# 2lambda123/CliMA-Oceananigans.jl

Hardware: AMD Instinct MI355X
Metric: cell-updates/sec per time_step!, 256^3 Nonhydrostatic WENO5 (higher is better)
Workload: dtype f64

## Files before the change

### clima-oceananigans.jl_amd/csrc/compat.h

```cpp
#pragma once

#include <cmath>
#include <cstddef>
#include <cstdint>
#include <cstdio>
#include <cstdlib>
#include <cstring>

#ifndef OCN_HOST_EMU
#include <hip/hip_runtime.h>
#include <hipfft/hipfft.h>

#define OCN_DEVFN __device__ __forceinline__

extern thread_local int g_ocn_dry;

struct ocn_launch_error {
  hipError_t err;
  char what[200];
};
extern thread_local ocn_launch_error g_ocn_launch_err;
static inline void ocn_note_error(hipError_t e, const char* what) {
  if (e == hipSuccess || g_ocn_launch_err.err != hipSuccess) return;
  g_ocn_launch_err.err = e;
// ... 14 lines not shown

typedef __attribute__((address_space(3))) void ocn_lds_void;
typedef const __attribute__((address_space(1))) void ocn_glb_void;
__device__ __forceinline__ void ocn_glds16(const void* src_lane, void* dst_wave_base, int ) {
  __builtin_amdgcn_global_load_lds((ocn_glb_void*)src_lane, (ocn_lds_void*)dst_wave_base, 16, 0, 0);
}
__device__ __forceinline__ double ocn_shfl_next(double x) {
  union { double d; int i[2]; } a, b;
  a.d = x;
  b.i[0] = __builtin_amdgcn_update_dpp(0, a.i[0], 0x130, 0xf, 0xf, false);
  b.i[1] = __builtin_amdgcn_update_dpp(0, a.i[1], 0x130, 0xf, 0xf, false);
  return b.d;
}
__device__ __forceinline__ double ocn_shfl_xor16(double x) {
  union { double d; int i[2]; } a, b;
  a.d = x;
  const int lane = __builtin_amdgcn_mbcnt_hi(~0u, __builtin_amdgcn_mbcnt_lo(~0u, 0u));
  const int addr = (lane ^ 16) << 2;
  b.i[0] = __builtin_amdgcn_ds_bpermute(addr, a.i[0]);
  b.i[1] = __builtin_amdgcn_ds_bpermute(addr, a.i[1]);
  return b.d;
}
#define OCN_WAVE 64
#define OCN_LD_NT(p) __builtin_nontemporal_load(p)
#define OCN_ST_NT(p, v) __builtin_nontemporal_store((v), (p))
#define OCN_UNIFORM(x) __builtin_amdgcn_readfirstlane(x)
typedef const __attribute__((address_space(4))) double ocn_const_double;
#define OCN_SLOAD(p) (*(ocn_const_double*)(p))

#else
#include <chrono>
#include <condition_variable>
#include <mutex>
#include <thread>
#include <vector>

struct dim3 {
  unsigned x, y, z;
  dim3(unsigned a = 1, unsigned b = 1, unsigned c = 1) : x(a), y(b), z(c) {}
};
extern thread_local dim3 threadIdx, blockIdx, blockDim, gridDim;
#define g_ocn_dry 0
extern std::recursive_mutex g_emu_launch_mutex;

#define __global__
#define __device__
// ... 50 lines not shown
          for (unsigned ty = 0; ty < block.y; ++ty)
            for (unsigned tx = 0; tx < block.x; ++tx) {
              threadIdx = dim3(tx, ty, tz);
              kern(args...);
            }
      }
}

struct emu_barrier {
  std::mutex m;
  std::condition_variable cv;
  unsigned count = 0, n = 0, gen = 0;
  void wait() {
    std::unique_lock<std::mutex> lk(m);
    unsigned g = gen;
    if (++count == n) { count = 0; ++gen; cv.notify_all(); }
    else cv.wait(lk, [&] { return g != gen; });
  }
};
extern emu_barrier g_emu_barrier;
static inline void __syncthreads() { g_emu_barrier.wait(); }

#define OCN_WAVE 64
#define OCN_UNIFORM(x) (x)
#define OCN_SLOAD(p) (*(p))
#define OCN_LD_NT(p) (*(p))
#define OCN_ST_NT(p, v) ((void)(*(p) = (v)))
static inline void ocn_glds16(const void* src_lane, void* dst_wave_base, int lane) {
  memcpy((char*)dst_wave_base + 16 * lane, src_lane, 16);
}
extern double g_emu_shfl[4096];
static inline double ocn_shfl_xor16(double x) {
  const unsigned tid = threadIdx.x + blockDim.x * (threadIdx.y + blockDim.y * threadIdx.z);
  g_emu_shfl[tid] = x;
  g_emu_barrier.wait();
  const double y = g_emu_shfl[tid ^ 16];
  g_emu_barrier.wait();
  return y;
}
static inline double ocn_shfl_next(double x) {
  const unsigned tid = threadIdx.x + blockDim.x * (threadIdx.y + blockDim.y * threadIdx.z);
  const unsigned n = blockDim.x * blockDim.y * blockDim.z;
  g_emu_shfl[tid] = x;
  g_emu_barrier.wait();
  const double y = ((tid & 63) != 63 && tid + 1 < n) ? g_emu_shfl[tid + 1] : 0.0;
  g_emu_barrier.wait();
// ... 38 lines not shown
```

### clima-oceananigans.jl_amd/csrc/fused.hip

```cpp
#include "internal.h"

#define FUSED_MAX_THREADS 1024

struct FusedArgs {
  const double *u, *v, *w;
  const double *gmu, *gmv, *gmw;
  double *gnu, *gnv, *gnw;
  double *us, *vs, *ws;
  unsigned org;
  double dt, cn, cm;
  int use_m;
  int BYo;
  int ntiles;
  int ntx, BXo;
  int prio;
  double nu;
  int zlo, zhi;
  int zlo2, zhi2;
  int gran;
};

#ifndef OCN_HOST_EMU
#define OCN_SETPRIO(n) __builtin_amdgcn_s_setprio(n)
#else
// ... 874 lines not shown
  if (m->d.closure == OCN_CLOSURE_AMD || m->d.closure == OCN_CLOSURE_SMAG || m->d.coriolis_fplane || m->d.buoyancy != OCN_BUOYANCY_NONE) return false;
  if (tiled_blocker(m)) return false;
  if (getenv("OCNHIP_NO_FUSED")) return false;
  return true;
}

bool fused_available(const ocn_model* m) {
  if (m->stokes) return false;
  return fused_available_but_for_stokes(m);
}

static bool tend4_asel(const ocn_model* m, bool plain);

void fused_describe(const ocn_model* m, char* buf, size_t n) {
  const char* why = tiled_blocker(m);
  if (m->fast_path) {
    const size_t halo_bytes = (size_t)(3 + m->nt) * m->gd.Hz * m->u.sz * sizeof(double);
    const bool ov = m->g->dist && m->gd.Nz > 2 * m->gd.Hz + 2 &&
                    (m->knob_overlap >= 0 ? m->knob_overlap != 0 : (m->ctx->nranks > 1 && halo_bytes >= ((size_t)8 << 20)));
    const bool asel = tend4_asel(m, !(m->d.closure == OCN_CLOSURE_SCALAR && m->d.nu != 0.0));
    const char* pform = m->g->dist ? "" : pnhs_lazy(m) ? " (pressure written on demand)"
                        : m->pnhs_escaped ? " (pressure stored by every projection: its device pointer was handed out)"
                                          : " (pressure stored by every projection)";
    snprintf(buf, n, "all-in-one periodic path: k_tend4%s + fused Poisson passes + k_project%s%s", asel ? " (address-selected stencils)" : "",
             pform, !m->g->dist ? "" : ov ? "; z-slabs, halo planes travel under the next interior tendency launch"
                                   : "; z-slabs, halo exchange on the model's stream");
  }
  else if (m->bz_fast) snprintf(buf, n, "tiled advection + update (k_tend4, REST) on top of the %s other terms",
                                rest4_ok(m) ? "tiled kernel's (k_rest4)" : "general kernels'");
  else if (why) snprintf(buf, n, "general kernels: %s", why);
  else if (m->g->topo[0] == OCN_FLAT || m->g->topo[1] == OCN_FLAT) snprintf(buf, n, "general kernels: Flat x / y slices are outside the tiled kernels");
  else snprintf(buf, n, "general kernels (tiled path disabled or not applicable to this topology / decomposition)");
  if (m->stokes && fused_available_but_for_stokes(m)) {
    const size_t l = strlen(buf);
    snprintf(buf + l, n - l, "; not the all-in-one periodic path: Stokes drift terms are served by %s",
             rest4_ok(m) ? "k_rest4" : "the general kernel");
  }
  if (m->d.closure == OCN_CLOSURE_SMAG) {
    const size_t l = strlen(buf);
    snprintf(buf + l, n - l, "; nu_e: %s", smag_tiled_ok(m) ? "tiled kernel (k_smag_nu)" : "one thread per cell (k_smag_nu_cell)");
  }
}

int fused_cu_count(const ocn_model* m) {
  static int ncu = 0;
  if (!ncu) {
#ifndef OCN_HOST_EMU
    hipDeviceProp_t prop;
    ncu = (hipGetDeviceProperties(&prop, m->ctx->device) == hipSuccess) ? prop.multiProcessorCount : 256;
#else
    ncu = 8;
#endif
  }
  return ncu;
}

struct FusedShape {
  int bx, by;
  bool wide, small;
  int dma;
  bool asel;
  dim3 blk, grd;
};

void fused_read_knobs(ocn_model* m) {
  auto env = [](const char* n, int def) { const char* e = getenv(n); return e ? atoi(e) : def; };
  m->knob_fused_xt = env("OCNHIP_FUSED_XT", 0);
  m->knob_no_dma = env("OCNHIP_NO_LDS_DMA", 0);
  m->knob_no_tracer3 = env("OCNHIP_NO_TRACER3", 0);
  m->knob_xfft_team = env("OCNHIP_XFFT_TEAM", 0);
  m->knob_overlap = env("OCNHIP_OVERLAP", -1);
  m->knob_overlap_cus = env("OCNHIP_OVERLAP_CUS", 16);
  m->knob_graph = env("OCNHIP_NO_GRAPH", 0) ? 0 : 1;
  { const char* e = getenv("OCNHIP_PRIO"); m->knob_prio = e ? (int)strtol(e, nullptr, 0) : 0x20FF; }
  { const char* e = getenv("OCNHIP_LOCALITY"); m->knob_locality = e ? atoi(e) : 1; }
  m->knob_no_smag_tiled = env("OCNHIP_NO_SMAG_TILED", 0);
  m->knob_tend4_vsel = env("OCNHIP_TEND4_VSEL", 0);
  m->knob_eager_pressure = env("OCNHIP_EAGER_PRESSURE", 0);
}

static bool tend4_asel(const ocn_model* m, bool plain) {
  const GridDev& gd = m->gd;
  if (!plain || m->knob_tend4_vsel || gd.Nx > 256 || gd.xb || (m->knob_fused_xt == 1 && gd.Nx <= 57 * 4)) return false;
#ifdef OCN_HOST_EMU
  return gd.Nx <= 16;
#else
  return gd.Nx > 128;
#endif
}

static FusedShape fused_shape(const ocn_model* m, FusedArgs& a, bool plain = false) {
  const GridDev& gd = m->gd;
  FusedShape f;
// ... 364 lines not shown
```

### clima-oceananigans.jl_amd/csrc/internal.h

```cpp
#pragma once
#include <map>
#include <string>
#include <vector>

#include "../../include/ocnhip.h"
#include "compat.h"
#include "stencils.h"

#define OCN_NF (3 + OCN_MAX_TRACERS)
#define OCN_CLOSURE_SMAG 3

struct ProfPhase {
  std::vector<std::pair<hipEvent_t, hipEvent_t>> ev;
  double total_ms = 0;
  int64_t count = 0;
};

struct ocn_ctx {
  int device = 0;
  hipStream_t stream = nullptr;
  char err[512] = {0};
  bool profiling = false;
  std::map<std::string, ProfPhase> prof;
  std::string prof_only;
// ... 73 lines not shown
  double time = 0, previous_dt = INFINITY;
  int64_t iteration = 0;
  int stage = 1;
  double* d_red = nullptr;
  int fast_path = 0;
  int bz_fast = 0;
  double* amd_tab = nullptr;
  double smag_C = 0, smag_Cb = 0, smag_rPr[OCN_MAX_TRACERS] = {0};
  double* smag_tab = nullptr;
  int knob_no_smag_tiled = 0;
  double* phi_below = nullptr;
  double *ypack_s = nullptr, *ypack_r = nullptr;
  size_t ypack_n = 0;
  bool gn_alias_gm = false;
  bool pred_active = false;
  ocn_grid* own_grid = nullptr;
  int knob_fused_xt = 0, knob_no_dma = 0, knob_no_tracer3 = 0, knob_prio = 0x20FF;
  struct StepGraph { uint64_t key; int seen; void* exec; std::vector<uint64_t> words; };
  std::vector<StepGraph> graphs;
  int knob_overlap_cus = 16;
  int knob_overlap = -1;
  bool halo_inflight = false, halo2_inflight = false;
  bool pnhs_halo_stale = false;
  int knob_xfft_team = 0;
  int knob_graph = 1;
  int knob_tend4_vsel = 0;
  int knob_locality = 1;
  bool pnhs_deferred = false;
  bool pnhs_escaped = false;
  int knob_eager_pressure = 0;
  int stokes = 0;
  double* stokes_dev = nullptr;
  double* stokes_stage = nullptr;
  hipEvent_t stokes_ev[3] = {nullptr, nullptr, nullptr};
  bool graph_off = false;
  int64_t graph_replays = 0;
};
extern thread_local int g_ocn_capturing, g_ocn_capture_poison;
inline Field& pred_u(ocn_model* m) { return m->pred_active ? m->us : m->u; }
inline Field& pred_v(ocn_model* m) { return m->pred_active ? m->vs : m->v; }
inline Field& pred_w(ocn_model* m) { return m->pred_active ? m->ws : m->w; }
inline bool pnhs_lazy(const ocn_model* m) { return m->fast_path && !m->g->dist && !m->knob_eager_pressure && !m->pnhs_escaped; }

inline const double* stokes_slot(const ocn_model* m) {
  return m->stokes ? m->stokes_dev + (size_t)(m->stage - 1) * 6 * m->gd.Nz : nullptr;
}
// ... 35 lines not shown
bool fused_tracer3_ok(const ocn_model* m);
bool tracer_rest_shell(const ocn_model* m);
void launch_tracer3(ocn_model* m, double dt, double cn, double cm, int use_m, bool rest);
void launch_fused_tend_step(ocn_model* m, double dt, double cn, double cm, int use_m, int zlo = 0, int zhi = -1, int zlo2 = 0, int zhi2 = 0);
void launch_rhs_wrap(ocn_model* m, double dt, double* rhs);
void launch_project(ocn_model* m, double dt, const double* phi, bool store_p = true);
void launch_pressure_images(ocn_model* m, const double* phi);
void launch_tracer_steps(ocn_model* m, double dt, double cn, double cm, int use_m);
int fused_exchange_ws(ocn_model* m);
int fused_exchange_phi(ocn_model* m, const double* phi);
int poisson_run(ocn_model* m);

PoissonSolver* poisson_create(ocn_model* m);
void poisson_destroy(PoissonSolver* s);
int poisson_solve(ocn_model* m, double dt);
int poisson_solve_rhs(ocn_model* m, const double* rhs_dev, double* phi_dev);
double* poisson_rhs_buffer(PoissonSolver* s);

void* zsolve_create(ocn_ctx* ctx, const std::vector<double>& lx_half, const std::vector<double>& ly_local);
void zsolve_destroy(void* z);
void zsolve_run(ocn_ctx* ctx, void* z, void* spec, int Nz, const double* lz, double norm, long zero_col);
void yfft_run(ocn_ctx* ctx, void* z, void* spec, int Nxh, int Ny, int Nz, int inverse);
void xfft_rhs_run(ocn_model* m, void* z, void* spec, double dt, int extra_plane = 0);
bool poisson_local_wstar(const ocn_model* m);
bool fft_size_ok(int n);
bool zsolve_size_ok(int n);
bool poisson_custom_xy(const ocn_model* m);
int poisson_run_from_predictor(ocn_model* m, double dt);

void* zslab_create(ocn_ctx* ctx, const std::vector<double>& lx_half, const std::vector<double>& ly, int n, int R, int rank);
void zslab_destroy(void* z);
int zslab_run(ocn_ctx* ctx, void* z, void* spec, double dz2, double scale, const void* below = nullptr, void* phi_below = nullptr);
bool poisson_local_phi_below(const ocn_model* m);
const double* poisson_phi_below(const ocn_model* m);

int comm_exchange(ocn_ctx* c, const std::vector<CommOp>& sends, const std::vector<CommOp>& recvs, hipStream_t st = nullptr);
int comm_halo_exchange_z(ocn_model* m, Field** fs, int n, hipStream_t st = nullptr);
bool comm_can_overlap(const ocn_ctx* c);
int halo_settle(ocn_model* m);
int comm_halo_exchange_y(ocn_model* m, Field** fs, int n);
int comm_alltoall(ocn_ctx* c, const void* send, void* recv, size_t block_bytes);
void comm_destroy(ocn_ctx* c);

struct ProfScope {
  ocn_ctx* c;
  hipEvent_t a = nullptr, b = nullptr;
// ... 5 lines not shown
```

### clima-oceananigans.jl_amd/csrc/poisson.hip

```cpp
#include "internal.h"
#ifndef OCN_HOST_EMU
#define dry_hipfftExecD2Z(...) (g_ocn_dry ? HIPFFT_SUCCESS : hipfftExecD2Z(__VA_ARGS__))
#define dry_hipfftExecZ2D(...) (g_ocn_dry ? HIPFFT_SUCCESS : hipfftExecZ2D(__VA_ARGS__))
#define dry_hipfftExecZ2Z(...) (g_ocn_dry ? HIPFFT_SUCCESS : hipfftExecZ2Z(__VA_ARGS__))
#endif


#ifndef OCN_HOST_EMU
#include <rocblas/rocblas.h>
#endif
#include <complex>
typedef std::complex<double> cplx;

struct double2_ {
  double x, y;
};

struct PoissonSolver {
  int kind;
  int Nx, Ny, Nz, Nxh;
  int R = 1, rank = 0, Nzg = 0, Nyl = 0;
  double2_ *ta = nullptr, *tb = nullptr;
  void* zs = nullptr;
  void* zsl = nullptr;
  double dz2 = 0;
  bool cxy = false;
  bool cxy_bz = false;
  double2_* bplane = nullptr;
  bool local_phi = false;
  void* tw = nullptr;
  double* rhs = nullptr;
  double2_* spec = nullptr;
  double* tscr = nullptr;
  int* tri_kbr = nullptr;
  bool tri_ready = false;
  double *lx = nullptr, *ly = nullptr, *lz = nullptr;
  bool tr = false;
  int gNx = 0, gNy = 0, gR = 0;
  int gtopo[2] = {0, 0};
  double *ra = nullptr, *rb = nullptr;
  double2_ *ga = nullptr, *gb = nullptr;
  double* gm[2][2] = {{nullptr, nullptr}, {nullptr, nullptr}};
  void* blas = nullptr;
  int yw = 0, Nyg = 0;
  double2_ *ysend = nullptr, *yrecv = nullptr, *yT = nullptr;
#ifndef OCN_HOST_EMU
  hipfftHandle fwd = 0, inv = 0, zplan = 0, xinv = 0;
  hipfftHandle wxf = 0, wxi = 0, wz = 0;
  hipfftHandle yfft = 0;
// ... 57 lines not shown
    if (rc5) {
      poisson_destroy(s);
      return nullptr;
    }
    return s;
  }
  if (g->topo[0] != OCN_PERIODIC || g->topo[1] != OCN_PERIODIC) {
    s->kind = 4;
    int rc4 = walls_create(m, s);
    if (rc4) {
      poisson_destroy(s);
      return nullptr;
    }
    return s;
  }
  if (g->dist) {
    s->kind = 2;
    s->R = m->ctx->nranks;
    s->rank = m->ctx->rank;
    s->Nzg = g->Nzg;
    s->Nyl = s->Ny / s->R;
  }
  size_t nr = (size_t)s->Nx * s->Ny * s->Nz, nc = (size_t)s->Nxh * s->Ny * s->Nz;
  const size_t xr = g->dist ? (size_t)s->Nx * s->Ny : 0, xc = g->dist ? (size_t)s->Nxh * s->Ny : 0;
  if (hipMalloc((void**)&s->rhs, (nr + xr) * sizeof(double)) != hipSuccess ||
      hipMalloc((void**)&s->spec, (nc + xc) * sizeof(double2_)) != hipSuccess) {
    poisson_destroy(s);
    return nullptr;
  }
  if (g->topo[2] == OCN_BOUNDED) {
    if (hipMalloc((void**)&s->tscr, 2 * (size_t)s->Nxh * s->Ny * s->Nz * sizeof(double)) != hipSuccess ||
        hipMalloc((void**)&s->tri_kbr, (size_t)s->Nxh * s->Ny * sizeof(int)) != hipSuccess) {
      poisson_destroy(s);
      return nullptr;
    }
  }
  const char* dsolver = getenv("OCNHIP_DIST_SOLVER");
  const bool use_slab = g->dist && !(dsolver && strcmp(dsolver, "transpose") == 0);
  if (use_slab) {
    std::vector<double> lxh = eigenvalues_periodic(s->Nx, g->L[0]);
    lxh.resize(s->Nxh);
    s->zsl = zslab_create(m->ctx, lxh, eigenvalues_periodic(s->Ny, g->L[1]), s->Nz, s->R, s->rank);
    if (!s->zsl) {
      poisson_destroy(s);
      return nullptr;
    }
// ... 6 lines not shown
    std::vector<double> lxh = eigenvalues_periodic(s->Nx, g->L[0]);
    lxh.resize(s->Nxh);
    std::vector<double> lyv = eigenvalues_periodic(s->Ny, g->L[1]);
    if (g->dist) lyv = std::vector<double>(lyv.begin() + s->rank * s->Nyl, lyv.begin() + (s->rank + 1) * s->Nyl);
    s->zs = zsolve_create(m->ctx, lxh, lyv);
    if (!s->zs) {
      poisson_destroy(s);
      return nullptr;
    }
    if (s->kind == 0) s->kind = 3;
  }
  if (fft_size_ok(s->Nx) && fft_size_ok(s->Ny) && g->topo[2] == OCN_PERIODIC && g->z_regular &&
      !(getenv("OCNHIP_NO_CUSTOM_XY") && atoi(getenv("OCNHIP_NO_CUSTOM_XY")) != 0)) {
    if (!s->zs && !s->zsl) {
      std::vector<double> lxh = eigenvalues_periodic(s->Nx, g->L[0]);
      lxh.resize(s->Nxh);
      s->zsl = zslab_create(m->ctx, lxh, eigenvalues_periodic(s->Ny, g->L[1]), s->Nz, 1, 0);
      double dz = g->L[2] / g->Nzg;
      s->dz2 = dz * dz;
    }
    std::vector<double> one(1, 0.0);
    s->tw = zsolve_create(m->ctx, one, one);
    s->cxy = s->tw != nullptr && (s->zs || s->zsl);
    if (s->cxy && g->dist && s->zsl && !(getenv("OCNHIP_WSTAR_EXCHANGE") && atoi(getenv("OCNHIP_WSTAR_EXCHANGE")) != 0)) {
      s->bplane = s->spec + nc;
      s->local_phi = !(getenv("OCNHIP_PHI_EXCHANGE") && atoi(getenv("OCNHIP_PHI_EXCHANGE")) != 0);
    }
  }
  if (g->topo[2] == OCN_BOUNDED && s->kind == 1 && fft_size_ok(s->Nx) && fft_size_ok(s->Ny) && g->topo[0] == OCN_PERIODIC &&
      g->topo[1] == OCN_PERIODIC && s->Nx + 2 * g->PH[0] == (int)m->gd.sy &&
      !(getenv("OCNHIP_NO_CUSTOM_XY") && atoi(getenv("OCNHIP_NO_CUSTOM_XY")) != 0)) {
    std::vector<double> one(1, 0.0);
    s->tw = zsolve_create(m->ctx, one, one);
    s->cxy_bz = s->tw != nullptr;
  }
  s->lx = upload(eigenvalues_periodic(s->Nx, g->L[0]));
  s->ly = upload(eigenvalues_periodic(s->Ny, g->L[1]));
  if (g->topo[2] == OCN_PERIODIC) s->lz = upload(eigenvalues_periodic(g->dist ? g->Nzg : s->Nz, g->L[2]));
  if (s->kind == 2 && !s->zsl) {
    if (hipMalloc((void**)&s->ta, nc * sizeof(double2_)) != hipSuccess ||
        hipMalloc((void**)&s->tb, nc * sizeof(double2_)) != hipSuccess) {
      poisson_destroy(s);
      return nullptr;
    }
  }
#ifndef OCN_HOST_EMU
// ... 813 lines not shown
      dim3 gr((s->Nxh + 63) / 64, (s->Ny + 3) / 4, s->Nz);
      double norm = 1.0 / ((double)s->Nx * s->Ny * (s->kind == 0 ? s->Nz : 1));
      ocn_launch(k_scale_spectrum, gr, b, st, s->Nxh, s->Ny, s->Nz, (const double*)s->lx, (const double*)s->ly,
                 (const double*)s->lz, norm, s->spec);
    }
  }
  {
    ProfScope ps(m->ctx, "fft_backward");
#ifndef OCN_HOST_EMU
    if (dry_hipfftExecZ2D(s->inv, (hipfftDoubleComplex*)s->spec, s->rhs) != HIPFFT_SUCCESS) {
      ocn_set_error(m->ctx, "hipfftExecZ2D failed");
      return OCN_EHIP;
    }
#else
    emu_backward(s);
#endif
  }
  return OCN_OK;
}

int poisson_run(ocn_model* m) { return run_solver(m); }

bool poisson_custom_xy(const ocn_model* m) { return m->solver && m->solver->cxy; }
bool poisson_local_wstar(const ocn_model* m) { return m->solver && m->solver->bplane != nullptr; }
bool poisson_local_phi_below(const ocn_model* m) { return m->solver && m->solver->bplane != nullptr && m->solver->local_phi; }
const double* poisson_phi_below(const ocn_model* m) { return m->solver->rhs + (size_t)m->solver->Nx * m->solver->Ny * m->solver->Nz; }

#ifdef OCN_HOST_EMU
static void emu_xinv(PoissonSolver* s, const double2_* spec = nullptr, double* out = nullptr, size_t nlines = 0) {
  const int Nx = s->Nx, Nxh = s->Nxh;
  const size_t lines = nlines ? nlines : (size_t)s->Ny * s->Nz;
  if (!spec) spec = s->spec;
  if (!out) out = s->rhs;
  std::vector<cplx> full(Nx);
  for (size_t L = 0; L < lines; ++L) {
    for (int i = 0; i < Nx; ++i) {
      double2_ q = spec[(i < Nxh ? i : Nx - i) + Nxh * L];
      full[i] = cplx(q.x, i < Nxh ? q.y : -q.y);
    }
    for (int n = 0; n < Nx; ++n) {
      cplx acc = 0;
      for (int i = 0; i < Nx; ++i) {
        double ang = 2.0 * M_PI * ((long)i * n % Nx) / Nx;
        acc += full[i] * cplx(cos(ang), sin(ang));
      }
      out[n + Nx * L] = acc.real();
    }
  }
}
#endif

int poisson_run_from_predictor(ocn_model* m, double dt) {
  PoissonSolver* s = m->solver;
  const int xp = s->bplane ? 1 : 0, ip = (s->bplane && s->local_phi) ? 1 : 0;
  {
    ProfScope ps(m->ctx, "fft_forward");
    xfft_rhs_run(m, s->tw, s->spec, dt, xp);
    yfft_run(m->ctx, s->tw, s->spec, s->Nxh, s->Ny, s->Nz + xp, 0);
  }
  if (s->zs) {
    ProfScope ps(m->ctx, "spectral_solve");
    zsolve_run(m->ctx, s->zs, s->spec, s->Nz, s->lz, 1.0 / ((double)s->Nx * s->Ny * s->Nz), 0);
  } else {
    int rc = zslab_run(m->ctx, s->zsl, s->spec, s->dz2, 1.0 / ((double)s->Nx * s->Ny), s->bplane, ip ? s->bplane : nullptr);
    if (rc) return rc;
  }
  {
    ProfScope ps(m->ctx, "fft_backward");
    yfft_run(m->ctx, s->tw, s->spec, s->Nxh, s->Ny, s->Nz + ip, 1);
#ifndef OCN_HOST_EMU
    if (dry_hipfftExecZ2D(s->xinv, (hipfftDoubleComplex*)s->spec, s->rhs) != HIPFFT_SUCCESS) {
      ocn_set_error(m->ctx, "hipfftExecZ2D (x inverse) failed");
      return OCN_EHIP;
    }
#else
    emu_xinv(s, s->spec, s->rhs, (size_t)s->Ny * (s->Nz + ip));
// ... 67 lines not shown
```

### clima-oceananigans.jl_amd/csrc/zfft.hip

```cpp
#include "internal.h"

struct cd {
  double x, y;
};
OCN_DEVFN cd cadd(cd a, cd b) { return {a.x + b.x, a.y + b.y}; }
OCN_DEVFN cd csub(cd a, cd b) { return {a.x - b.x, a.y - b.y}; }
OCN_DEVFN cd cmul(cd a, cd b) { return {a.x * b.x - a.y * b.y, a.x * b.y + a.y * b.x}; }
template <int S> OCN_DEVFN cd mul_mi(cd a) { return S > 0 ? cd{a.y, -a.x} : cd{-a.y, a.x}; }

template <int S> OCN_DEVFN void dft4(cd& a, cd& b, cd& c, cd& d) {
  cd s0 = cadd(a, c), s1 = csub(a, c), s2 = cadd(b, d), s3 = mul_mi<S>(csub(b, d));
  a = cadd(s0, s2);
  c = csub(s0, s2);
  b = cadd(s1, s3);
  d = csub(s1, s3);
}

template <int S> OCN_DEVFN void dft16(cd* v) {
#pragma unroll
  for (int a = 0; a < 4; ++a) dft4<S>(v[a], v[a + 4], v[a + 8], v[a + 12]);
  const double C1 = 0.92387953251128673848, S1 = 0.38268343236508978178, R = 0.70710678118654752440;
  auto tw = [&](cd z, double c, double s) { return cd{z.x * c + S * z.y * s, z.y * c - S * z.x * s}; };
  v[1 + 4] = tw(v[1 + 4], C1, S1);
  v[1 + 8] = tw(v[1 + 8], R, R);
// ... 12 lines not shown
    for (int d = c + 1; d < 4; ++d) {
      cd t = v[4 * c + d];
      v[4 * c + d] = v[4 * d + c];
      v[4 * d + c] = t;
    }
}

template <int S> OCN_DEVFN void dft8(cd* v) {
  cd e0 = v[0], e1 = v[2], e2 = v[4], e3 = v[6], o0 = v[1], o1 = v[3], o2 = v[5], o3 = v[7];
  dft4<S>(e0, e1, e2, e3);
  dft4<S>(o0, o1, o2, o3);
  const double R = 0.70710678118654752440;
  auto tw = [&](cd z, double c, double s) { return cd{z.x * c + S * z.y * s, z.y * c - S * z.x * s}; };
  o1 = tw(o1, R, R);
  o2 = mul_mi<S>(o2);
  o3 = tw(o3, -R, R);
  v[0] = cadd(e0, o0); v[4] = csub(e0, o0);
  v[1] = cadd(e1, o1); v[5] = csub(e1, o1);
  v[2] = cadd(e2, o2); v[6] = csub(e2, o2);
  v[3] = cadd(e3, o3); v[7] = csub(e3, o3);
}

#define SMN (16 * (256 + 32))
template <int N> struct FftGeo {
  static constexpr int M = N / 16;
  static constexpr int C = 256 / M;
  static constexpr int CS = N == 512 ? 16 : C;
  static constexpr int RS = N == 128 ? 8 : 16;
  static constexpr int K1S = RS * CS + CS;
};

template <int N, int S, bool XL = false> OCN_DEVFN void fft_stage2(double* sm, cd* v, int r, int c, const cd* tw) {
  typedef FftGeo<N> G;
  constexpr int KX = G::RS * G::CS + 1;
  constexpr int TS = 512 / (N == 512 ? 256 : N);
#pragma unroll
  for (int k1 = 1; k1 < 16; ++k1) {
    cd w = tw[((r * k1) * TS) & 511];
    if (S < 0) w.y = -w.y;
    v[k1] = cmul(v[k1], w);
  }
  auto wi = [&](int k1) { return XL ? k1 * KX + c * G::RS + r : k1 * G::K1S + r * G::CS + c; };
  if (N == 128) {
    auto ri = [&](int q) {
      return XL ? (r + 8 * (q >> 3)) * KX + c * G::RS + (q & 7) : (r + 8 * (q >> 3)) * G::K1S + (q & 7) * G::CS + c;
    };
#pragma unroll
    for (int q = 0; q < 16; ++q) sm[wi(q)] = v[q].x;
    __syncthreads();
#pragma unroll
    for (int q = 0; q < 16; ++q) v[q].x = sm[ri(q)];
    __syncthreads();
#pragma unroll
    for (int q = 0; q < 16; ++q) sm[wi(q)] = v[q].y;
    __syncthreads();
#pragma unroll
    for (int q = 0; q < 16; ++q) v[q].y = sm[ri(q)];
    dft8<S>(v);
    dft8<S>(v + 8);
  } else {
    auto ri = [&](int n2) { return XL ? r * KX + c * G::RS + n2 : r * G::K1S + n2 * G::CS + c; };
#pragma unroll
    for (int q = 0; q < 16; ++q) sm[wi(q)] = v[q].x;
    __syncthreads();
#pragma unroll
    for (int q = 0; q < 16; ++q) v[q].x = sm[ri(q)];
    __syncthreads();
#pragma unroll
    for (int q = 0; q < 16; ++q) sm[wi(q)] = v[q].y;
    __syncthreads();
#pragma unroll
    for (int q = 0; q < 16; ++q) v[q].y = sm[ri(q)];
    dft16<S>(v);
  }
}

OCN_DEVFN void fft512_partner(double* sm, const cd* v, cd* p, int r, int c) {
  const int me = r * 16 + c, other = r * 16 + (c ^ 8);
  __syncthreads();
#pragma unroll
  for (int q = 0; q < 16; ++q) sm[q * 256 + me] = v[q].x;
  __syncthreads();
#pragma unroll
  for (int q = 0; q < 16; ++q) p[q].x = sm[q * 256 + other];
  __syncthreads();
#pragma unroll
  for (int q = 0; q < 16; ++q) sm[q * 256 + me] = v[q].y;
  __syncthreads();
#pragma unroll
  for (int q = 0; q < 16; ++q) p[q].y = sm[q * 256 + other];
  __syncthreads();
}

template <int N, int S, bool XLANE = false> OCN_DEVFN void fft_fwd(double* sm, cd* v, int r, int c, const cd* tw) {
  if (N == 512) {
    cd p[16];
    if (XLANE) {
#pragma unroll
      for (int q = 0; q < 16; ++q) p[q] = cd{ocn_shfl_xor16(v[q].x), 0.0};
    } else fft512_partner(sm, v, p, r, c);
    const int h = (c >> 3) & 1;
#pragma unroll
    for (int n1 = 0; n1 < 16; ++n1) {
      if (h == 0) v[n1] = cadd(v[n1], p[n1]);
      else {
        cd w = tw[(r + 16 * n1) & 511];
        if (S < 0) w.y = -w.y;
        v[n1] = cmul(csub(p[n1], v[n1]), w);
      }
    }
  }
  dft16<S>(v);
  fft_stage2<N, S, XLANE>(sm, v, r, c, tw);
}

template <int N> OCN_DEVFN void fft_back(double* sm, cd* v, int r, int c, const cd* tw) {
  typedef FftGeo<N> G;
  constexpr int TS = 512 / (N == 512 ? 256 : N);
  if (N == 128) {
    dft8<-1>(v);
    dft8<-1>(v + 8);
#pragma unroll
    for (int q = 0; q < 16; ++q) {
      cd w = tw[(((r + 8 * (q >> 3)) * (q & 7)) * TS) & 511];
      w.y = -w.y;
      v[q] = cmul(v[q], w);
    }
    auto wi = [&](int q) { return (r + 8 * (q >> 3)) * G::K1S + (q & 7) * G::CS + c; };
    auto ri = [&](int k1) { return k1 * G::K1S + r * G::CS + c; };
    __syncthreads();
#pragma unroll
    for (int q = 0; q < 16; ++q) sm[wi(q)] = v[q].x;
    __syncthreads();
#pragma unroll
    for (int q = 0; q < 16; ++q) v[q].x = sm[ri(q)];
    __syncthreads();
#pragma unroll
    for (int q = 0; q < 16; ++q) sm[wi(q)] = v[q].y;
    __syncthreads();
#pragma unroll
// ... 4 lines not shown
  dft16<-1>(v);
#pragma unroll
  for (int n2 = 1; n2 < 16; ++n2) {
    cd w = tw[((r * n2) * TS) & 511];
    w.y = -w.y;
    v[n2] = cmul(v[n2], w);
  }
  auto wi = [&](int n2) { return r * G::K1S + n2 * G::CS + c; };
  auto ri = [&](int k1) { return k1 * G::K1S + r * G::CS + c; };
  __syncthreads();
#pragma unroll
  for (int q = 0; q < 16; ++q) sm[wi(q)] = v[q].x;
  __syncthreads();
#pragma unroll
  for (int q = 0; q < 16; ++q) v[q].x = sm[ri(q)];
  __syncthreads();
#pragma unroll
  for (int q = 0; q < 16; ++q) sm[wi(q)] = v[q].y;
  __syncthreads();
#pragma unroll
  for (int q = 0; q < 16; ++q) v[q].y = sm[ri(q)];
  dft16<-1>(v);
  if (N == 512) {
    const int h = (c >> 3) & 1;
    if (h == 1) {
#pragma unroll
      for (int n1 = 0; n1 < 16; ++n1) {
        cd w = tw[(r + 16 * n1) & 511];
        w.y = -w.y;
        v[n1] = cmul(v[n1], w);
      }
    }
    cd p[16];
    fft512_partner(sm, v, p, r, c);
#pragma unroll
    for (int n1 = 0; n1 < 16; ++n1) v[n1] = h == 0 ? cadd(v[n1], p[n1]) : csub(p[n1], v[n1]);
  }
}

template <int N> OCN_DEVFN void team_of(int t, int& r, int& c, int& col) {
  typedef FftGeo<N> G;
  c = t % G::CS;
  r = t / G::CS;
  col = N == 512 ? (c & 7) : c;
}
template <int N> OCN_DEVFN int pos_in(int r, int c, int n1) {
  return N == 128 ? r + 8 * n1 : N == 256 ? r + 16 * n1 : r + 16 * n1 + 256 * ((c >> 3) & 1);
}
template <int N> OCN_DEVFN int pos_out(int r, int c, int q) {
  return N == 128 ? (r + 8 * (q >> 3)) + 16 * (q & 7) : N == 256 ? r + 16 * q : 2 * (r + 16 * q) + ((c >> 3) & 1);
}

template <int N>
__global__ void __launch_bounds__(256) k_zsolve(cd* __restrict__ a, long ncol, const double* __restrict__ lxy,
                                                const double* __restrict__ lz, const cd* __restrict__ tw, double norm, long zero_col) {
  OCN_SHARED double sm[SMN];
  int r, c, col;
  team_of<N>(threadIdx.x, r, c, col);
  const long gcol = (long)blockIdx.x * FftGeo<N>::C + col;
  const bool ok = gcol < ncol;
  cd v[16];
#pragma unroll
  for (int n1 = 0; n1 < 16; ++n1) v[n1] = ok ? a[gcol + ncol * pos_in<N>(r, c, n1)] : cd{0, 0};
  fft_fwd<N, 1>(sm, v, r, c, tw);
  const double lc = ok ? lxy[gcol] : 1.0;
#pragma unroll
  for (int q = 0; q < 16; ++q) {
    const int kz = pos_out<N>(r, c, q);
    double f = -norm / (lc + lz[kz]);
    if (gcol == zero_col && kz == 0) f = 0.0;
    v[q].x *= f;
    v[q].y *= f;
  }
// ... 229 lines not shown
      const int ie = (i + 1 == g.Nx) ? 0 : i + 1;
      double d = 0.0;
      if (ok && extra && k == g.Nz) d = ws[j * sy + i] * rdz * rdt;
      else if (ok && g.zb) {
        const double dzc = g_dzc(g, k);
        d = ((us[row + ie] - us[row + i]) * g.rdx + (vs[rown + i] - vs[row + i]) * g.rdy + (ws[rowt + i] - ws[row + i]) / dzc) * rdt * dzc;
      } else if (ok) d = ((us[row + ie] - us[row + i]) * g.rdx + (vs[rown + i] - vs[row + i]) * g.rdy + (ws[rowt + i] - ws[row + i]) * rdz) * rdt;
      v[n1] = {d, 0.0};
    }
  }
  fft_fwd<N, 1, true>(sm, v, r, c, tw);
  if (ok) {
    cd* out = spec + L * (N / 2 + 1);
#pragma unroll
    for (int q = 0; q < 16; ++q) {
      const int kmin = N == 128 ? 8 * (q >> 3) + 16 * (q & 7) : N == 256 ? 16 * q : 32 * q;
      if (kmin > N / 2) continue;
      const int kx = pos_out<N>(r, c, q);
      if (kx <= N / 2) out[kx] = v[q];
    }
  }
}

struct ZSolve {
  cd* twmr = nullptr;
  int twmr_n = 0;
  cd* tw = nullptr;
  double* lxy = nullptr;
  long ncol = 0;
};

bool fft_size_ok(int n) { return n == 128 || n == 256 || n == 512; }
bool zsolve_size_ok(int n) { return fft_size_ok(n) || n == 320 || n == 384; }

void* zsolve_create(ocn_ctx* ctx, const std::vector<double>& lx_half, const std::vector<double>& ly_local) {
  ZSolve* z = new ZSolve;
  const size_t Nxh = lx_half.size(), Ny = ly_local.size();
  z->ncol = (long)(Nxh * Ny);
  std::vector<double> lxy(Nxh * Ny);
  for (size_t j = 0; j < Ny; ++j)
    for (size_t i = 0; i < Nxh; ++i) lxy[i + Nxh * j] = lx_half[i] + ly_local[j];
  std::vector<cd> tw(512);
  for (int m = 0; m < 512; ++m) tw[m] = {cos(2.0 * M_PI * m / 512.0), -sin(2.0 * M_PI * m / 512.0)};
  if (hipMalloc((void**)&z->tw, sizeof(cd) * 512) != hipSuccess ||
      hipMalloc((void**)&z->lxy, sizeof(double) * lxy.size()) != hipSuccess) {
    ocn_set_error(ctx, "zsolve: allocation failed");
// ... 74 lines not shown
        ocn_set_error(ctx, "zsolve: allocation failed");
        return;
      }
      hipMemcpy(z->twmr, t.data(), sizeof(cd) * Nz, hipMemcpyHostToDevice);
      z->twmr_n = Nz;
    }
    dim3 g((unsigned)((z->ncol + 15) / 16), 1, 1);
    cd* a = (cd*)spec;
    if (Nz == 320)
      ocn_launch_sync(k_zsolve_mr<20>, g, dim3(320, 1, 1), ctx->stream, a, z->ncol, (const double*)z->lxy, lz, (const cd*)z->twmr, norm, zero_col);
    else
      ocn_launch_sync(k_zsolve_mr<24>, g, dim3(384, 1, 1), ctx->stream, a, z->ncol, (const double*)z->lxy, lz, (const cd*)z->twmr, norm, zero_col);
    return;
  }
  const int C = 256 / (Nz / 16);
  dim3 b(256, 1, 1), g((unsigned)((z->ncol + C - 1) / C), 1, 1);
  cd* a = (cd*)spec;
  const cd* tw = (const cd*)z->tw;
  hipStream_t s = ctx->stream;
  FFT_BY_N(Nz, ocn_launch_sync(k_zsolve<128>, g, b, s, a, z->ncol, (const double*)z->lxy, lz, tw, norm, zero_col),
           ocn_launch_sync(k_zsolve<256>, g, b, s, a, z->ncol, (const double*)z->lxy, lz, tw, norm, zero_col),
           ocn_launch_sync(k_zsolve<512>, g, b, s, a, z->ncol, (const double*)z->lxy, lz, tw, norm, zero_col))
}
```

Baseline: 16.68 billion.

## Split the y-FFT across x and z Poisson passes for a three-pass solve

```diff
diff --git a/clima-oceananigans.jl_amd/csrc/compat.h b/clima-oceananigans.jl_amd/csrc/compat.h
--- a/clima-oceananigans.jl_amd/csrc/compat.h
+++ b/clima-oceananigans.jl_amd/csrc/compat.h
@@ -60,6 +60,12 @@
   return b.d;
 }
 #define OCN_WAVE 64
+#define OCN_WAVE_SYNC()                                      \
+  do {                                                       \
+    __builtin_amdgcn_fence(__ATOMIC_RELEASE, "wavefront");   \
+    __builtin_amdgcn_wave_barrier();                         \
+    __builtin_amdgcn_fence(__ATOMIC_ACQUIRE, "wavefront");   \
+  } while (0)
 #define OCN_LD_NT(p) __builtin_nontemporal_load(p)
 #define OCN_ST_NT(p, v) __builtin_nontemporal_store((v), (p))
 #define OCN_UNIFORM(x) __builtin_amdgcn_readfirstlane(x)
@@ -156,6 +162,7 @@
 static inline void __syncthreads() { g_emu_barrier.wait(); }
 
 #define OCN_WAVE 64
+#define OCN_WAVE_SYNC() g_emu_barrier.wait()
 #define OCN_UNIFORM(x) (x)
 #define OCN_SLOAD(p) (*(p))
 #define OCN_LD_NT(p) (*(p))
diff --git a/clima-oceananigans.jl_amd/csrc/fused.hip b/clima-oceananigans.jl_amd/csrc/fused.hip
--- a/clima-oceananigans.jl_amd/csrc/fused.hip
+++ b/clima-oceananigans.jl_amd/csrc/fused.hip
@@ -920,8 +920,9 @@
     const char* pform = m->g->dist ? "" : pnhs_lazy(m) ? " (pressure written on demand)"
                         : m->pnhs_escaped ? " (pressure stored by every projection: its device pointer was handed out)"
                                           : " (pressure stored by every projection)";
-    snprintf(buf, n, "all-in-one periodic path: k_tend4%s + fused Poisson passes + k_project%s%s", asel ? " (address-selected stencils)" : "",
-             pform, !m->g->dist ? "" : ov ? "; z-slabs, halo planes travel under the next interior tendency launch"
+    const char* yform = !poisson_custom_xy(m) || m->g->dist ? "" : poisson_split_y(m) ? " (split-y form: three passes)" : " (five-pass form)";
+    snprintf(buf, n, "all-in-one periodic path: k_tend4%s + fused Poisson passes%s + k_project%s%s", asel ? " (address-selected stencils)" : "",
+             yform, pform, !m->g->dist ? "" : ov ? "; z-slabs, halo planes travel under the next interior tendency launch"
                                    : "; z-slabs, halo exchange on the model's stream");
   }
   else if (m->bz_fast) snprintf(buf, n, "tiled advection + update (k_tend4, REST) on top of the %s other terms",
@@ -967,6 +968,7 @@
   m->knob_no_dma = env("OCNHIP_NO_LDS_DMA", 0);
   m->knob_no_tracer3 = env("OCNHIP_NO_TRACER3", 0);
   m->knob_xfft_team = env("OCNHIP_XFFT_TEAM", 0);
+  m->knob_split_y = env("OCNHIP_SPLIT_Y", 1);
   m->knob_overlap = env("OCNHIP_OVERLAP", -1);
   m->knob_overlap_cus = env("OCNHIP_OVERLAP_CUS", 16);
   m->knob_graph = env("OCNHIP_NO_GRAPH", 0) ? 0 : 1;
diff --git a/clima-oceananigans.jl_amd/csrc/internal.h b/clima-oceananigans.jl_amd/csrc/internal.h
--- a/clima-oceananigans.jl_amd/csrc/internal.h
+++ b/clima-oceananigans.jl_amd/csrc/internal.h
@@ -119,6 +119,7 @@
   int knob_overlap = -1;
   bool halo_inflight = false, halo2_inflight = false;
   bool pnhs_halo_stale = false;
+  int knob_split_y = 1;
   int knob_xfft_team = 0;
   int knob_graph = 1;
   int knob_tend4_vsel = 0;
@@ -200,6 +201,12 @@
 void zsolve_run(ocn_ctx* ctx, void* z, void* spec, int Nz, const double* lz, double norm, long zero_col);
 void yfft_run(ocn_ctx* ctx, void* z, void* spec, int Nxh, int Ny, int Nz, int inverse);
 void xfft_rhs_run(ocn_model* m, void* z, void* spec, double dt, int extra_plane = 0);
+bool split_y_ok(int Nx, int Ny, int Nz);
+int split_y_pitch(int Nx);
+void xfft_rhs_sy_run(ocn_model* m, void* tw, void* spec, double dt);
+void zsolve_sy_run(ocn_ctx* ctx, void* zs, void* spec, int Nx, int Nz, const double* lz, double norm);
+void xinv_sy_run(ocn_ctx* ctx, void* tw, const void* spec, double* real, int Nx, int Ny, int Nz);
+bool poisson_split_y(const ocn_model* m);
 bool poisson_local_wstar(const ocn_model* m);
 bool fft_size_ok(int n);
 bool zsolve_size_ok(int n);
diff --git a/clima-oceananigans.jl_amd/csrc/poisson.hip b/clima-oceananigans.jl_amd/csrc/poisson.hip
--- a/clima-oceananigans.jl_amd/csrc/poisson.hip
+++ b/clima-oceananigans.jl_amd/csrc/poisson.hip
@@ -25,6 +25,7 @@
   void* zsl = nullptr;
   double dz2 = 0;
   bool cxy = false;
+  bool split_y = false;
   bool cxy_bz = false;
   double2_* bplane = nullptr;
   bool local_phi = false;
@@ -128,6 +129,8 @@
     s->Nyl = s->Ny / s->R;
   }
   size_t nr = (size_t)s->Nx * s->Ny * s->Nz, nc = (size_t)s->Nxh * s->Ny * s->Nz;
+  const bool may_split = m->knob_split_y && !m->knob_xfft_team && !g->dist && g->topo[2] == OCN_PERIODIC && g->z_regular && split_y_ok(s->Nx, s->Ny, s->Nz);
+  if (may_split) nc = (size_t)split_y_pitch(s->Nx) * s->Ny * s->Nz;
   const size_t xr = g->dist ? (size_t)s->Nx * s->Ny : 0, xc = g->dist ? (size_t)s->Nxh * s->Ny : 0;
   if (hipMalloc((void**)&s->rhs, (nr + xr) * sizeof(double)) != hipSuccess ||
       hipMalloc((void**)&s->spec, (nc + xc) * sizeof(double2_)) != hipSuccess) {
@@ -180,6 +183,7 @@
     std::vector<double> one(1, 0.0);
     s->tw = zsolve_create(m->ctx, one, one);
     s->cxy = s->tw != nullptr && (s->zs || s->zsl);
+    s->split_y = may_split && s->cxy && s->zs;
     if (s->cxy && g->dist && s->zsl && !(getenv("OCNHIP_WSTAR_EXCHANGE") && atoi(getenv("OCNHIP_WSTAR_EXCHANGE")) != 0)) {
       s->bplane = s->spec + nc;
       s->local_phi = !(getenv("OCNHIP_PHI_EXCHANGE") && atoi(getenv("OCNHIP_PHI_EXCHANGE")) != 0);
@@ -1039,6 +1043,7 @@
 int poisson_run(ocn_model* m) { return run_solver(m); }
 
 bool poisson_custom_xy(const ocn_model* m) { return m->solver && m->solver->cxy; }
+bool poisson_split_y(const ocn_model* m) { return m->solver && m->solver->split_y; }
 bool poisson_local_wstar(const ocn_model* m) { return m->solver && m->solver->bplane != nullptr; }
 bool poisson_local_phi_below(const ocn_model* m) { return m->solver && m->solver->bplane != nullptr && m->solver->local_phi; }
 const double* poisson_phi_below(const ocn_model* m) { return m->solver->rhs + (size_t)m->solver->Nx * m->solver->Ny * m->solver->Nz; }
@@ -1069,6 +1074,21 @@
 
 int poisson_run_from_predictor(ocn_model* m, double dt) {
   PoissonSolver* s = m->solver;
+  if (s->split_y) {
+    {
+      ProfScope ps(m->ctx, "fft_forward");
+      xfft_rhs_sy_run(m, s->tw, s->spec, dt);
+    }
+    {
+      ProfScope ps(m->ctx, "spectral_solve");
+      zsolve_sy_run(m->ctx, s->zs, s->spec, s->Nx, s->Nz, s->lz, 1.0 / ((double)s->Nx * s->Ny * s->Nz));
+    }
+    {
+      ProfScope ps(m->ctx, "fft_backward");
+      xinv_sy_run(m->ctx, s->tw, s->spec, s->rhs, s->Nx, s->Ny, s->Nz);
+    }
+    return OCN_OK;
+  }
   const int xp = s->bplane ? 1 : 0, ip = (s->bplane && s->local_phi) ? 1 : 0;
   {
     ProfScope ps(m->ctx, "fft_forward");
diff --git a/clima-oceananigans.jl_amd/csrc/zfft.hip b/clima-oceananigans.jl_amd/csrc/zfft.hip
--- a/clima-oceananigans.jl_amd/csrc/zfft.hip
+++ b/clima-oceananigans.jl_amd/csrc/zfft.hip
@@ -58,16 +58,16 @@
 }
 
 #define SMN (16 * (256 + 32))
-template <int N> struct FftGeo {
+template <int N, int T = 256> struct FftGeo {
   static constexpr int M = N / 16;
-  static constexpr int C = 256 / M;
-  static constexpr int CS = N == 512 ? 16 : C;
+  static constexpr int C = T / M;
+  static constexpr int CS = N == 512 ? 2 * C : C;
   static constexpr int RS = N == 128 ? 8 : 16;
   static constexpr int K1S = RS * CS + CS;
 };
 
-template <int N, int S, bool XL = false> OCN_DEVFN void fft_stage2(double* sm, cd* v, int r, int c, const cd* tw) {
-  typedef FftGeo<N> G;
+template <int N, int S, bool XL = false, int T = 256> OCN_DEVFN void fft_stage2(double* sm, cd* v, int r, int c, const cd* tw) {
+  typedef FftGeo<N, T> G;
   constexpr int KX = G::RS * G::CS + 1;
   constexpr int TS = 512 / (N == 512 ? 256 : N);
 #pragma unroll
@@ -111,31 +111,44 @@
   }
 }
 
-OCN_DEVFN void fft512_partner(double* sm, const cd* v, cd* p, int r, int c) {
-  const int me = r * 16 + c, other = r * 16 + (c ^ 8);
-  __syncthreads();
-#pragma unroll
-  for (int q = 0; q < 16; ++q) sm[q * 256 + me] = v[q].x;
-  __syncthreads();
-#pragma unroll
-  for (int q = 0; q < 16; ++q) p[q].x = sm[q * 256 + other];
-  __syncthreads();
-#pragma unroll
-  for (int q = 0; q < 16; ++q) sm[q * 256 + me] = v[q].y;
-  __syncthreads();
-#pragma unroll
-  for (int q = 0; q < 16; ++q) p[q].y = sm[q * 256 + other];
-  __syncthreads();
-}
-
-template <int N, int S, bool XLANE = false> OCN_DEVFN void fft_fwd(double* sm, cd* v, int r, int c, const cd* tw) {
-  if (N == 512) {
+template <int T = 256> OCN_DEVFN void fft512_partner(double* sm, const cd* v, cd* p, int r, int c) {
+  constexpr int C = FftGeo<512, T>::C;
+  const int me = r * 2 * C + c, other = r * 2 * C + (c ^ C);
+  __syncthreads();
+#pragma unroll
+  for (int q = 0; q < 16; ++q) sm[q * T + me] = v[q].x;
+  __syncthreads();
+#pragma unroll
+  for (int q = 0; q < 16; ++q) p[q].x = sm[q * T + other];
+  __syncthreads();
+#pragma unroll
+  for (int q = 0; q < 16; ++q) sm[q * T + me] = v[q].y;
+  __syncthreads();
+#pragma unroll
+  for (int q = 0; q < 16; ++q) p[q].y = sm[q * T + other];
+  __syncthreads();
+}
+
+template <int N, int S, bool XLANE = false, int T = 256, bool CPLX = false> OCN_DEVFN void fft_fwd(double* sm, cd* v, int r, int c, const cd* tw) {
+  if (N == 512 && XLANE && CPLX) {
+    const int h = (c / FftGeo<512, T>::C) & 1;
+#pragma unroll
+    for (int n1 = 0; n1 < 16; ++n1) {
+      const cd p = cd{ocn_shfl_xor16(v[n1].x), ocn_shfl_xor16(v[n1].y)};
+      if (h == 0) v[n1] = cadd(v[n1], p);
+      else {
+        cd w = tw[(r + 16 * n1) & 511];
+        if (S < 0) w.y = -w.y;
+        v[n1] = cmul(csub(p, v[n1]), w);
+      }
+    }
+  } else if (N == 512) {
     cd p[16];
     if (XLANE) {
 #pragma unroll
       for (int q = 0; q < 16; ++q) p[q] = cd{ocn_shfl_xor16(v[q].x), 0.0};
-    } else fft512_partner(sm, v, p, r, c);
-    const int h = (c >> 3) & 1;
+    } else fft512_partner<T>(sm, v, p, r, c);
+    const int h = (c / FftGeo<512, T>::C) & 1;
 #pragma unroll
     for (int n1 = 0; n1 < 16; ++n1) {
       if (h == 0) v[n1] = cadd(v[n1], p[n1]);
@@ -147,11 +160,11 @@
     }
   }
   dft16<S>(v);
-  fft_stage2<N, S, XLANE>(sm, v, r, c, tw);
-}
-
-template <int N> OCN_DEVFN void fft_back(double* sm, cd* v, int r, int c, const cd* tw) {
-  typedef FftGeo<N> G;
+  fft_stage2<N, S, XLANE, T>(sm, v, r, c, tw);
+}
+
+template <int N, int T = 256> OCN_DEVFN void fft_back(double* sm, cd* v, int r, int c, const cd* tw) {
+  typedef FftGeo<N, T> G;
   constexpr int TS = 512 / (N == 512 ? 256 : N);
   if (N == 128) {
     dft8<-1>(v);
@@ -202,7 +215,7 @@
   for (int q = 0; q < 16; ++q) v[q].y = sm[ri(q)];
   dft16<-1>(v);
   if (N == 512) {
-    const int h = (c >> 3) & 1;
+    const int h = (c / FftGeo<512, T>::C) & 1;
     if (h == 1) {
 #pragma unroll
       for (int n1 = 0; n1 < 16; ++n1) {
@@ -212,23 +225,23 @@
       }
     }
     cd p[16];
-    fft512_partner(sm, v, p, r, c);
+    fft512_partner<T>(sm, v, p, r, c);
 #pragma unroll
     for (int n1 = 0; n1 < 16; ++n1) v[n1] = h == 0 ? cadd(v[n1], p[n1]) : csub(p[n1], v[n1]);
   }
 }
 
-template <int N> OCN_DEVFN void team_of(int t, int& r, int& c, int& col) {
-  typedef FftGeo<N> G;
+template <int N, int T = 256> OCN_DEVFN void team_of(int t, int& r, int& c, int& col) {
+  typedef FftGeo<N, T> G;
   c = t % G::CS;
   r = t / G::CS;
-  col = N == 512 ? (c & 7) : c;
-}
-template <int N> OCN_DEVFN int pos_in(int r, int c, int n1) {
-  return N == 128 ? r + 8 * n1 : N == 256 ? r + 16 * n1 : r + 16 * n1 + 256 * ((c >> 3) & 1);
-}
-template <int N> OCN_DEVFN int pos_out(int r, int c, int q) {
-  return N == 128 ? (r + 8 * (q >> 3)) + 16 * (q & 7) : N == 256 ? r + 16 * q : 2 * (r + 16 * q) + ((c >> 3) & 1);
+  col = N == 512 ? c % G::C : c;
+}
+template <int N, int T = 256> OCN_DEVFN int pos_in(int r, int c, int n1) {
+  return N == 128 ? r + 8 * n1 : N == 256 ? r + 16 * n1 : r + 16 * n1 + 256 * ((c / FftGeo<N, T>::C) & 1);
+}
+template <int N, int T = 256> OCN_DEVFN int pos_out(int r, int c, int q) {
+  return N == 128 ? (r + 8 * (q >> 3)) + 16 * (q & 7) : N == 256 ? r + 16 * q : 2 * (r + 16 * q) + ((c / FftGeo<N, T>::C) & 1);
 }
 
 template <int N>
@@ -504,6 +517,208 @@
   }
 }
 
+#define SY_R1 32
+#define SY_R2 8
+int split_y_pitch(int Nx) { return Nx / 2 + 8; }
+bool split_y_ok(int Nx, int Ny, int Nz) { return Ny == SY_R1 * SY_R2 && fft_size_ok(Nx) && fft_size_ok(Nz); }
+
+OCN_DEVFN long sy_at(int P, int kx, int k1, int ry, long k) { return kx + (long)P * (k1 + SY_R1 * (ry + SY_R2 * k)); }
+
+template <int S> OCN_DEVFN void dft32_half(cd* v, int p, const cd* tw) {
+  if (p) {
+#pragma unroll
+    for (int k = 1; k < 16; ++k) {
+      cd w = tw[16 * k];
+      if (S < 0) w.y = -w.y;
+      v[k] = cmul(v[k], w);
+    }
+  }
+  dft16<S>(v);
+}
+
+template <int N>
+__global__ void __launch_bounds__(2 * N) k_xfft_rhs_sy(GridDev g, const double* __restrict__ us, const double* __restrict__ vs,
+                                                       const double* __restrict__ ws, double rdt, int zwrap,
+                                                       cd* __restrict__ spec, const cd* __restrict__ tw) {
+  constexpr int T = 2 * N, M = N / 16, NH = N / 2 + 1, P = N / 2 + 8;
+  OCN_SHARED double sm[SMN * (T / 256)];
+  const int t = threadIdx.x;
+  const int rr = t % M, ln = t / M;
+  const int r = N == 512 ? rr & 15 : rr;
+  const int c = N == 512 ? ln + SY_R1 * (rr >> 4) : ln;
+  const int b = blockIdx.x;
+  const int ry = (b / 8) % SY_R2, k = (b / (8 * SY_R2)) * 8 + b % 8;
+  const long sy = g.sy, sz = g.sz;
+  const double rdz = 1.0 / g.dz;
+  constexpr int LP = N + 16;
+  static_assert(SY_R1 * LP <= SMN * (T / 256) && 2 * SY_R1 * NH <= SMN * (T / 256), "tiles must fit the transform's LDS buffer");
+  cd v[16];
+#pragma unroll
+  for (int m = 0; m < 16; ++m) {
+    const int e = t + T * m;
+    const int l2 = e / N, i = e - l2 * N;
+    const int j = ry + SY_R2 * l2;
+    const long row = j * sy + k * sz;
+    const long rown = ((j + 1 == g.Ny) ? 0 : j + 1) * sy + k * sz;
+    const long rowt = (zwrap && k + 1 == g.Nz) ? j * sy : j * sy + (k + 1) * sz;
+    const int ie = (i + 1 == g.Nx) ? 0 : i + 1;
+    sm[l2 * LP + i] = ((us[row + ie] - us[row + i]) * g.rdx + (vs[rown + i] - vs[row + i]) * g.rdy + (ws[rowt + i] - ws[row + i]) * rdz) * rdt;
+  }
+  __syncthreads();
+#pragma unroll
+  for (int n1 = 0; n1 < 16; ++n1) v[n1] = {sm[ln * LP + pos_in<N, T>(r, c, n1)], 0.0};
+  __syncthreads();
+  fft_fwd<N, 1, true, T>(sm, v, r, c, tw);
+  __syncthreads();
+  cd* ls = (cd*)sm;
+#pragma unroll
+  for (int q = 0; q < 16; ++q) {
+    const int kmin = N == 128 ? 8 * (q >> 3) + 16 * (q & 7) : N == 256 ? 16 * q : 32 * q;
+    if (kmin > N / 2) continue;
+    const int kx = pos_out<N, T>(r, c, q);
+    if (kx <= N / 2) ls[ln * NH + kx] = v[q];
+  }
+  __syncthreads();
+  const int p = t / NH, kx = t - p * NH;
+  if (p < 2) {
+#pragma unroll
+    for (int q = 0; q < 16; ++q) {
+      const cd a = ls[q * NH + kx], bb = ls[(q + 16) * NH + kx];
+      v[q] = p ? csub(a, bb) : cadd(a, bb);
+    }
+    dft32_half<1>(v, p, tw);
+#pragma unroll
+    for (int m = 0; m < 16; ++m) {
+      const int k1 = p + 2 * m;
+      spec[sy_at(P, kx, k1, ry, k)] = cmul(v[m], tw[(2 * ry * k1) & 511]);
+    }
+  }
+}
+
+template <int S, int T> OCN_DEVFN void sy_stage2(double* sm, cd* v, int t, int cw, int ry) {
+  constexpr int ST = T + 2;
+  const int t0 = t - cw * ry;
+  const int lv = 2 * ry;
+  cd u[16];
+  __syncthreads();
+#pragma unroll
+  for (int n1 = 0; n1 < 16; ++n1) sm[n1 * ST + t] = v[n1].x;
+  OCN_WAVE_SYNC();
+#pragma unroll
+  for (int q = 0; q < 16; ++q) u[q].x = sm[(lv + (q >> 3)) * ST + t0 + cw * (q & 7)];
+  OCN_WAVE_SYNC();
+#pragma unroll
+  for (int n1 = 0; n1 < 16; ++n1) sm[n1 * ST + t] = v[n1].y;
+  OCN_WAVE_SYNC();
+#pragma unroll
+  for (int q = 0; q < 16; ++q) u[q].y = sm[(lv + (q >> 3)) * ST + t0 + cw * (q & 7)];
+  dft8<S>(u);
+  dft8<S>(u + 8);
+  OCN_WAVE_SYNC();
+#pragma unroll
+  for (int q = 0; q < 16; ++q) sm[(lv + (q >> 3)) * ST + t0 + cw * (q & 7)] = u[q].x;
+  OCN_WAVE_SYNC();
+#pragma unroll
+  for (int n1 = 0; n1 < 16; ++n1) v[n1].x = sm[n1 * ST + t];
+  OCN_WAVE_SYNC();
+#pragma unroll
+  for (int q = 0; q < 16; ++q) sm[(lv + (q >> 3)) * ST + t0 + cw * (q & 7)] = u[q].y;
+  OCN_WAVE_SYNC();
+#pragma unroll
+  for (int n1 = 0; n1 < 16; ++n1) v[n1].y = sm[n1 * ST + t];
+  __syncthreads();
+}
+
+template <int N, int T>
+__global__ void __launch_bounds__(T) k_zsolve_sy(cd* __restrict__ a, int Nxh, int P, const double* __restrict__ lxy,
+                                                 const double* __restrict__ lz, const cd* __restrict__ tw, double norm) {
+  typedef FftGeo<N, T> G;
+  constexpr int CW = G::C / SY_R2;
+  static_assert(G::CS <= 64 && 16 * (T + 2) <= SMN * (T / 256), "the residues of a column group must be lanes of one wave");
+  OCN_SHARED double sm[SMN * (T / 256)];
+  int r, c, col;
+  team_of<N, T>(threadIdx.x, r, c, col);
+  const int kxs = col % CW, ry = col / CW;
+  const int tiles = (Nxh + CW - 1) / CW;
+  const int nblk = SY_R1 * tiles;
+  const int b = ((int)blockIdx.x % 8) * (nblk / 8) + (int)blockIdx.x / 8;
+  const int tile = b % tiles, k1 = b / tiles;
+  const int kx = tile * CW + kxs;
+  const bool ok = kx < Nxh;
+  const long ncol = (long)P * SY_R1 * SY_R2;
+  cd* col0 = a + sy_at(P, kx, k1, ry, 0);
+  cd v[16];
+#pragma unroll
+  for (int n1 = 0; n1 < 16; ++n1) v[n1] = ok ? col0[ncol * pos_in<N, T>(r, c, n1)] : cd{0, 0};
+  sy_stage2<1, T>(sm, v, threadIdx.x, CW, ry);
+  fft_fwd<N, 1, false, T>(sm, v, r, c, tw);
+  const int ky = k1 + SY_R1 * ry;
+  const double lc = ok ? lxy[kx + (long)Nxh * ky] : 1.0;
+#pragma unroll
+  for (int q = 0; q < 16; ++q) {
+    const int kz = pos_out<N, T>(r, c, q);
+    double f = -norm / (lc + lz[kz]);
+    if (kx == 0 && ky == 0 && kz == 0) f = 0.0;
+    v[q].x *= f;
+    v[q].y *= f;
+  }
+  fft_back<N, T>(sm, v, r, c, tw);
+  sy_stage2<-1, T>(sm, v, threadIdx.x, CW, ry);
+  if (ok) {
+#pragma unroll
+    for (int n1 = 0; n1 < 16; ++n1) col0[ncol * pos_in<N, T>(r, c, n1)] = v[n1];
+  }
+}
+
+template <int N>
+__global__ void __launch_bounds__(2 * N) k_xinv_sy(const cd* __restrict__ spec, double* __restrict__ real, int Ny,
+                                                   const cd* __restrict__ tw) {
+  constexpr int T = 2 * N, M = N / 16, NH = N / 2 + 1, P = N / 2 + 8, LP = N + 16;
+  OCN_SHARED double sm[SMN * (T / 256)];
+  const int t = threadIdx.x;
+  const int rr = t % M, ln = t / M;
+  const int r = N == 512 ? rr & 15 : rr;
+  const int c = N == 512 ? ln + SY_R1 * (rr >> 4) : ln;
+  const int b = blockIdx.x;
+  const int ry = b % SY_R2, k = b / SY_R2;
+  cd* ls = (cd*)sm;
+  cd v[16];
+  const int p = t / NH, kx = t - p * NH;
+  if (p < 2) {
+#pragma unroll
+    for (int q = 0; q < 16; ++q) {
+      cd w0 = tw[(2 * ry * q) & 511], w1 = tw[(2 * ry * (q + 16)) & 511];
+      w0.y = -w0.y;
+      w1.y = -w1.y;
+      const cd z0 = cmul(spec[sy_at(P, kx, q, ry, k)], w0), z1 = cmul(spec[sy_at(P, kx, q + 16, ry, k)], w1);
+      v[q] = p ? csub(z0, z1) : cadd(z0, z1);
+    }
+    dft32_half<-1>(v, p, tw);
+#pragma unroll
+    for (int m = 0; m < 16; ++m) ls[(p + 2 * m) * NH + kx] = v[m];
+  }
+  __syncthreads();
+#pragma unroll
+  for (int n1 = 0; n1 < 16; ++n1) {
+    const int i = pos_in<N, T>(r, c, n1);
+    const cd z = ls[ln * NH + (i <= N / 2 ? i : N - i)];
+    v[n1] = i <= N / 2 ? z : cd{z.x, -z.y};
+  }
+  __syncthreads();
+  fft_fwd<N, -1, true, T, true>(sm, v, r, c, tw);
+  __syncthreads();
+#pragma unroll
+  for (int q = 0; q < 16; ++q) sm[ln * LP + pos_out<N, T>(r, c, q)] = v[q].x;
+  __syncthreads();
+  double* out = real + (long)N * ((long)Ny * k + ry);
+#pragma unroll
+  for (int m = 0; m < 16; ++m) {
+    const int e = t + T * m;
+    const int l2 = e / N, i = e - l2 * N;
+    out[(long)N * SY_R2 * l2 + i] = sm[l2 * LP + i];
+  }
+}
+
 struct ZSolve {
   cd* twmr = nullptr;
   int twmr_n = 0;
@@ -624,3 +839,42 @@
            ocn_launch_sync(k_zsolve<256>, g, b, s, a, z->ncol, (const double*)z->lxy, lz, tw, norm, zero_col),
            ocn_launch_sync(k_zsolve<512>, g, b, s, a, z->ncol, (const double*)z->lxy, lz, tw, norm, zero_col))
 }
+
+void xfft_rhs_sy_run(ocn_model* m, void* p, void* spec, double dt) {
+  ZSolve* z = (ZSolve*)p;
+  const GridDev& g = m->gd;
+  const double* us = (m->fast_path ? m->us : pred_u(m)).interior();
+  const double* vs = (m->fast_path ? m->vs : pred_v(m)).interior();
+  const double* ws = (m->fast_path ? m->ws : pred_w(m)).interior();
+  dim3 gr((unsigned)(SY_R2 * g.Nz), 1, 1);
+  hipStream_t s = m->ctx->stream;
+  cd* sp = (cd*)spec;
+  const cd* tw = (const cd*)z->tw;
+  FFT_BY_N(g.Nx, ocn_launch_sync(k_xfft_rhs_sy<128>, gr, dim3(256, 1, 1), s, g, us, vs, ws, 1.0 / dt, 1, sp, tw),
+           ocn_launch_sync(k_xfft_rhs_sy<256>, gr, dim3(512, 1, 1), s, g, us, vs, ws, 1.0 / dt, 1, sp, tw),
+           ocn_launch_sync(k_xfft_rhs_sy<512>, gr, dim3(1024, 1, 1), s, g, us, vs, ws, 1.0 / dt, 1, sp, tw))
+}
+
+void zsolve_sy_run(ocn_ctx* ctx, void* p, void* spec, int Nx, int Nz, const double* lz, double norm) {
+  ZSolve* z = (ZSolve*)p;
+  const int Nxh = Nx / 2 + 1, P = split_y_pitch(Nx);
+  cd* a = (cd*)spec;
+  const cd* tw = (const cd*)z->tw;
+  const double* lxy = (const double*)z->lxy;
+  hipStream_t s = ctx->stream;
+  const unsigned t4 = (unsigned)(SY_R1 * ((Nxh + 3) / 4)), t2 = (unsigned)(SY_R1 * ((Nxh + 1) / 2));
+  FFT_BY_N(Nz, ocn_launch_sync(k_zsolve_sy<128, 256>, dim3(t4, 1, 1), dim3(256, 1, 1), s, a, Nxh, P, lxy, lz, tw, norm),
+           ocn_launch_sync(k_zsolve_sy<256, 512>, dim3(t4, 1, 1), dim3(512, 1, 1), s, a, Nxh, P, lxy, lz, tw, norm),
+           ocn_launch_sync(k_zsolve_sy<512, 512>, dim3(t2, 1, 1), dim3(512, 1, 1), s, a, Nxh, P, lxy, lz, tw, norm))
+}
+
+void xinv_sy_run(ocn_ctx* ctx, void* p, const void* spec, double* real, int Nx, int Ny, int Nz) {
+  ZSolve* z = (ZSolve*)p;
+  dim3 gr((unsigned)(SY_R2 * Nz), 1, 1);
+  hipStream_t s = ctx->stream;
+  const cd* sp = (const cd*)spec;
+  const cd* tw = (const cd*)z->tw;
+  FFT_BY_N(Nx, ocn_launch_sync(k_xinv_sy<128>, gr, dim3(256, 1, 1), s, sp, real, Ny, tw),
+           ocn_launch_sync(k_xinv_sy<256>, gr, dim3(512, 1, 1), s, sp, real, Ny, tw),
+           ocn_launch_sync(k_xinv_sy<512>, gr, dim3(1024, 1, 1), s, sp, real, Ny, tw))
+}
```

Result: faster. 17.26 billion (median of 6 runs) (+3.5%).
